# theori-io/nrsc5

Hardware: NVIDIA H100
Metric: cu8 I/Q Msamples/s (higher is better)
Workload: dtype u8/int16/f32

## Files before the change

### include/nrsc5_b200.h

```cpp
#ifndef NRSC5_B200_H
#define NRSC5_B200_H

#include <stddef.h>
#include <stdint.h>

#ifdef __cplusplus
extern "C" {
#endif

#define NRSC5B_MODE_FM 0
#define NRSC5B_MODE_AM 1

enum {
    NRSC5B_OK = 0,
    NRSC5B_ENODEV = -1,
    NRSC5B_EINVAL = -2,
    NRSC5B_ENOMEM = -3,
    NRSC5B_ECUDA = -4,
    NRSC5B_EFULL = -5,
    NRSC5B_EOVERFLOW = -6,
};

enum {
    NRSC5B_REC_FRAME = 1,
    NRSC5B_REC_PIDS = 2,
    NRSC5B_REC_SYNC = 3,
    NRSC5B_REC_LOST_SYNC = 4,
    NRSC5B_REC_MER = 5,
    NRSC5B_REC_BER = 6,
    NRSC5B_REC_SOFT_PM = 8,
    NRSC5B_REC_BLOCK = 9,
    NRSC5B_REC_PAD = 12,
    NRSC5B_REC_L2 = 20,
};

typedef struct nrsc5b_engine nrsc5b_engine_t;

typedef struct {
    int device;
    int nstreams;
    int mode;
    size_t input_capacity;
    size_t log_capacity;
    int emit_soft;
    int input_cs16;
} nrsc5b_config_t;

int nrsc5b_create(nrsc5b_engine_t **out, const nrsc5b_config_t *cfg);
void nrsc5b_destroy(nrsc5b_engine_t *e);
int nrsc5b_reset(nrsc5b_engine_t *e, int stream);
int nrsc5b_rewind(nrsc5b_engine_t *e);

int nrsc5b_set_cuda_stream(nrsc5b_engine_t *e, void *cuda_stream);

int nrsc5b_push_cu8(nrsc5b_engine_t *e, int stream, const uint8_t *buf, size_t nbytes);
int nrsc5b_push_cs16(nrsc5b_engine_t *e, int stream, const int16_t *buf, size_t nvalues);
int nrsc5b_push_cu8_all(nrsc5b_engine_t *e, const uint8_t *host, size_t host_stride, size_t nbytes);
int nrsc5b_push_cu8_device(nrsc5b_engine_t *e, int stream, const void *dev_buf, size_t nbytes);
int nrsc5b_attach_device_input(nrsc5b_engine_t *e, const void *dev_buf, size_t stride, size_t nbytes);

int nrsc5b_attach_device_log(nrsc5b_engine_t *e, void *dev_buf, size_t stride);

int nrsc5b_process(nrsc5b_engine_t *e);
int nrsc5b_process_available(nrsc5b_engine_t *e);
int nrsc5b_push_fence(nrsc5b_engine_t *e);
int nrsc5b_process_fence(nrsc5b_engine_t *e, int token);
int nrsc5b_prepare_async(nrsc5b_engine_t *e);
int nrsc5b_stage_cu8(nrsc5b_engine_t *e, int stream, const uint8_t *buf, size_t nbytes);
int nrsc5b_stage_cs16(nrsc5b_engine_t *e, int stream, const int16_t *buf, size_t nvalues);
int nrsc5b_submit(nrsc5b_engine_t *e, int flush);
int nrsc5b_poll(nrsc5b_engine_t *e, int wait);
const uint8_t *nrsc5b_batch_records(nrsc5b_engine_t *e, int stream, size_t *nbytes);

long nrsc5b_drain(nrsc5b_engine_t *e, int stream, uint8_t *out, size_t cap, size_t *needed);
int nrsc5b_drain_all(nrsc5b_engine_t *e, uint8_t *out, size_t out_stride, size_t *sizes);
int nrsc5b_take_overflow(nrsc5b_engine_t *e, int stream);
int nrsc5b_synchronize(nrsc5b_engine_t *e);

int nrsc5b_set_sync_state(nrsc5b_engine_t *e, int stream, int state);

typedef struct {
    uint64_t blocks;
    uint64_t samples;
    uint64_t p1_frames;
    uint64_t kernel_launches;
    uint64_t p1_fallbacks;
    uint64_t log_overflows;
} nrsc5b_stats_t;
int nrsc5b_get_stats(nrsc5b_engine_t *e, nrsc5b_stats_t *st);

int nrsc5b_set_profiling(nrsc5b_engine_t *e, int on);
int nrsc5b_get_kernel_times(nrsc5b_engine_t *e, double *ms4, unsigned long long *n4);

int nrsc5b_get_phase_cycles(nrsc5b_engine_t *e, unsigned long long *cyc12, unsigned long long *n12);

int nrsc5b_get_am_phase_cycles(nrsc5b_engine_t *e, unsigned long long *cyc12);

int nrsc5b_debug_set(int flags);

int nrsc5b_enable_l2(nrsc5b_engine_t *e, int on);

int nrsc5b_halfband_fm(int device, const uint8_t *cu8, size_t npairs, int16_t *out_ri);
int nrsc5b_viterbi_k7(int device, const int8_t *in, uint8_t *out, int len, int nframes);
int nrsc5b_viterbi_k7_ex(int device, const int8_t *in, uint8_t *out, int len, int nframes, int *fallbacks);
int nrsc5b_rs_decode(int device, uint8_t *blocks255, int *rc, int nblocks);
int nrsc5b_viterbi_k9(int device, const int8_t *in, uint8_t *out, int len, int njobs, unsigned g0, unsigned g1, unsigned g2,
                      int warmup, int chunk_warmup, int *rounds);
long nrsc5b_l2_frames(int device, const uint8_t *frames, size_t nbytes, uint8_t *out, size_t cap, size_t *needed);
int nrsc5b_fft2048(int device, const float *in, float *out, int nffts);

typedef struct nrsc5b_channelizer nrsc5b_channelizer_t;
int nrsc5b_chan_create(nrsc5b_channelizer_t **out, int device, const int *offsets_100khz, int nch);
void nrsc5b_chan_destroy(nrsc5b_channelizer_t *c);
int nrsc5b_chan_tables(nrsc5b_channelizer_t *c, int16_t *taps, int16_t *phasor);
int nrsc5b_chan_make_tables(const int *offsets_100khz, int nch, int16_t *taps, int16_t *phasor);
long long nrsc5b_chan_outputs(size_t nbytes);
int nrsc5b_chan_run_device(nrsc5b_channelizer_t *c, const void *d_cu8, size_t nbytes, void *d_out, size_t out_stride, void *cuda_stream);
int nrsc5b_chan_run(nrsc5b_channelizer_t *c, const uint8_t *cu8, size_t nbytes, int16_t *out);
int nrsc5b_chan_reset(nrsc5b_channelizer_t *c);
int nrsc5b_chan_push(nrsc5b_channelizer_t *c, const uint8_t *cu8, size_t nbytes, void *d_out, size_t out_stride, void *cuda_stream,
                     long long *nout);
int nrsc5b_chan_feed(nrsc5b_channelizer_t *c, nrsc5b_engine_t *e, const int *streams, const uint8_t *cu8, size_t nbytes);

int nrsc5b_chan_create_cs16(nrsc5b_channelizer_t **out, int device, const int *offsets_100khz, int nch);
int nrsc5b_chan_run_cs16(nrsc5b_channelizer_t *c, const int16_t *cs16, size_t nvalues, int16_t *out);
int nrsc5b_chan_run_device_cs16(nrsc5b_channelizer_t *c, const void *d_cs16, size_t nvalues, void *d_out, size_t out_stride,
                                void *cuda_stream);
int nrsc5b_chan_push_cs16(nrsc5b_channelizer_t *c, const int16_t *cs16, size_t nvalues, void *d_out, size_t out_stride,
                          void *cuda_stream, long long *nout);
int nrsc5b_chan_feed_cs16(nrsc5b_channelizer_t *c, nrsc5b_engine_t *e, const int *streams, const int16_t *cs16, size_t nvalues);

int nrsc5b_chan_create_am(nrsc5b_channelizer_t **out, int device, const int *offsets_10khz, int nch);
int nrsc5b_chan_create_am_cs16(nrsc5b_channelizer_t **out, int device, const int *offsets_10khz, int nch);
int nrsc5b_chan_make_tables_am(const int *offsets_10khz, int nch, int16_t *taps, int16_t *phasor);
long long nrsc5b_chan_outputs_am(size_t nbytes);

const char *nrsc5b_version(void);

#ifdef __cplusplus
}
#endif
#endif
```

### nrsc5_b200/csrc/engine.cu

```cuda
#include <cmath>
#include <cstdio>
#include <cstdlib>
#include <cstring>
#include <ctime>
#include <new>
#include <vector>

#include "../../include/nrsc5_b200.h"
#include "chan_feed.h"
#include "common.cuh"
#if defined(NB_EMU)
struct NvtxRange { explicit NvtxRange(const char *) {} };
#else
#include <nvtx3/nvToolsExt.h>
struct NvtxRange {
    explicit NvtxRange(const char *name) { nvtxRangePushA(name); }
    ~NvtxRange() { nvtxRangePop(); }
};
#endif
#include "rs.cuh"
#include "viterbi.cuh"
#include "viterbi_chunk.cuh"
#include "viterbi64.cuh"
#include "front.cuh"
// ... 1953 lines not shown
        }
    }
    CK(cudaStreamSynchronize(e->stream));
    return rc ? rc : (truncated ? NRSC5B_EOVERFLOW : NRSC5B_OK);
}

extern "C" int nrsc5b_take_overflow(nrsc5b_engine_t *e, int stream)
{
    if (!e || stream < 0 || stream >= e->dims.nstreams) return NRSC5B_EINVAL;
    const int v = e->overflowed[stream];
    e->overflowed[stream] = 0;
    return v;
}

extern "C" int nrsc5b_set_sync_state(nrsc5b_engine_t *e, int stream, int state)
{
    if (!e || stream < 0 || stream >= e->dims.nstreams || state < 0 || state > 2) return NRSC5B_EINVAL;
    CK(cudaMemcpyAsync(reinterpret_cast<uint8_t *>(e->dp.st + stream) + offsetof(StreamState, force_state), &state,
                       sizeof(int), cudaMemcpyHostToDevice, e->stream));
    CK(cudaStreamSynchronize(e->stream));
    return NRSC5B_OK;
}

extern "C" int nrsc5b_get_stats(nrsc5b_engine_t *e, nrsc5b_stats_t *out)
{
    if (!e || !out) return NRSC5B_EINVAL;
    CK(cudaStreamSynchronize(e->stream));
    const int S = e->dims.nstreams;
    CK(cudaMemcpy(e->h_state, e->dp.st, sizeof(StreamState) * S, cudaMemcpyDeviceToHost));
    unsigned long long frames = 0, samples = 0, blocks = 0, fb = 0;
    for (int s = 0; s < S; s++) {
        fb += e->h_state[s].p1_fallbacks;
        frames += e->h_state[s].frames_done;
        blocks += e->h_state[s].blocks_done;
        samples += (unsigned long long)(2 * e->h_state[s].start);
    }
    e->stats.p1_frames = frames;
    e->stats.p1_fallbacks = fb;
    e->stats.blocks = blocks;
    e->stats.samples = samples;
    *out = e->stats;
    return NRSC5B_OK;
}

static int use_device(int device)
{
    int ndev = 0;
    if (cudaGetDeviceCount(&ndev) != cudaSuccess || ndev <= 0 || device >= ndev) {
        fprintf(stderr, "nrsc5_b200: no usable CUDA device (the engine has no CPU path)\n");
        return NRSC5B_ENODEV;
    }
    if (cudaSetDevice(device) != cudaSuccess) return NRSC5B_ENODEV;
    return upload_tables(device);
}

extern "C" int nrsc5b_halfband_fm(int device, const uint8_t *cu8, size_t npairs, int16_t *out)
{
    int rc = use_device(device);
    if (rc) return rc;
    uint8_t *din = nullptr;
    short2 *dout = nullptr;
    CK(cudaMalloc(&din, 4 * npairs + 64));
    CK(cudaMalloc(&dout, npairs * sizeof(short2)));
    CK(cudaMemcpy(din, cu8, 4 * npairs, cudaMemcpyHostToDevice));
    launch_halfband_test(din, (long long)npairs, dout, 0);
    CK(cudaMemcpy(out, dout, npairs * sizeof(short2), cudaMemcpyDeviceToHost));
    cudaFree(din);
    cudaFree(dout);
    return NRSC5B_OK;
}

static int viterbi_k7_impl(int device, const int8_t *in, uint8_t *out, int len, int nframes, int *fallbacks);

extern "C" int nrsc5b_viterbi_k7(int device, const int8_t *in, uint8_t *out, int len, int nframes)
{
    return viterbi_k7_impl(device, in, out, len, nframes, nullptr);
}

extern "C" int nrsc5b_viterbi_k7_ex(int device, const int8_t *in, uint8_t *out, int len, int nframes, int *fallbacks)
{
    return viterbi_k7_impl(device, in, out, len, nframes, fallbacks);
}

static int viterbi_k7_impl(int device, const int8_t *in, uint8_t *out, int len, int nframes, int *fallbacks)
{
    int rc = use_device(device);
    if (rc) return rc;
    if (len < 32 || nframes <= 0) return NRSC5B_EINVAL;
    int8_t *din = nullptr;
    uint8_t *dout = nullptr;
    size_t nin = (size_t)nframes * 3 * len;
    CK(cudaMalloc(&din, nin));
    CK(cudaMalloc(&dout, (size_t)nframes * len));
    CK(cudaMemcpy(din, in, nin, cudaMemcpyHostToDevice));
    if (len >= 2048 && (len % 32) == 0) {
        const int total = len + 64;
        int *dflags = nullptr;
        CK(cudaMalloc(&dflags, (size_t)nframes * 3 * sizeof(int)));
        std::vector<int> fl(3 * (size_t)nframes, 0);
        for (int i = 0; i < nframes; i++) fl[i] = 1;
        CK(cudaMemcpy(dflags, fl.data(), fl.size() * sizeof(int), cudaMemcpyHostToDevice));
        uint32_t *dbw = nullptr;
        CK(cudaMalloc(&dbw, (size_t)nframes * (len / 32) * sizeof(uint32_t)));
        VitcArgs a;
        a.len = len;
        a.nch = (total + CH_LEN - 1) / CH_LEN;
        a.dec_stride = (size_t)a.nch * CH_LEN;
        a.ready_stride = 1;
        CK(cudaMalloc(&a.dec, (size_t)nframes * a.dec_stride * sizeof(uint2)));
        CK(cudaMalloc(&a.vspec, (size_t)nframes * a.nch * 16 * sizeof(uint2)));
        CK(cudaMalloc(&a.vend, (size_t)nframes * a.nch * 16 * sizeof(uint2)));
        CK(cudaMalloc(&a.tbend, (size_t)nframes * a.nch * sizeof(int)));
        CK(cudaMalloc(&a.hstate, (size_t)nframes * a.nch * sizeof(int)));
        a.vin = din;
        a.bitsw = dbw;
        a.ready = dflags + 2 * nframes;
        a.slow = dflags + nframes;
        V64Args b;
        b.vin = din;
        b.dec = a.dec;
        b.bitsw = dbw;
        b.ready = dflags;
        b.retry = dflags + 2 * nframes;
        b.stride = 1;
        b.len = len;
        b.ch = len >= 16384 ? 1024 : 256;
        b.nch = (total + b.ch - 1) / b.ch;
        b.dec_stride = a.dec_stride;
        CK(cudaMalloc(&b.vspec, (size_t)nframes * b.nch * 32 * sizeof(uint32_t)));
        CK(cudaMalloc(&b.vend, (size_t)nframes * b.nch * 32 * sizeof(uint32_t)));
        CK(cudaMalloc(&b.endstate, (size_t)nframes * sizeof(int)));
        CK(cudaFuncSetAttribute(k_vitc_emit, cudaFuncAttributeMaxDynamicSharedMemorySize, (int)vitc_emit_smem()));
        CK(cudaFuncSetAttribute(k_v64_emit, cudaFuncAttributeMaxDynamicSharedMemorySize, (int)V64_EMIT_SMEM));
        launch_v64(b, nframes, 0);
        launch_vitc(a, nframes, 0);
        {
            size_t nb = (size_t)nframes * len;
            k_vitc_unpack<<<(unsigned)((nb + 255) / 256), 256>>>(dbw, dout, nb);
        }
        CK(cudaDeviceSynchronize());
        CK(cudaMemcpy(fl.data(), dflags, fl.size() * sizeof(int), cudaMemcpyDeviceToHost));
        if (fallbacks) {
            *fallbacks = 0;
            for (int i = 0; i < nframes; i++) *fallbacks += fl[2 * (size_t)nframes + i] != 0;
        }
        cudaFree(a.dec); cudaFree(a.vspec); cudaFree(a.vend); cudaFree(a.tbend); cudaFree(a.hstate); cudaFree(dflags); cudaFree(dbw);
        cudaFree(b.vspec); cudaFree(b.vend); cudaFree(b.endstate);
    } else {
        uint2 *ddec = nullptr;
        CK(cudaMalloc(&ddec, (size_t)nframes * (len + 64) * sizeof(uint2)));
        k_viterbi_test<<<nframes, 32>>>(din, dout, ddec, len);
        CK(cudaDeviceSynchronize());
        cudaFree(ddec);
    }
    CK(cudaMemcpy(out, dout, (size_t)nframes * len, cudaMemcpyDeviceToHost));
    cudaFree(din);
    cudaFree(dout);
    return NRSC5B_OK;
}

extern "C" int nrsc5b_rs_decode(int device, uint8_t *blocks, int *rcs, int n)
{
    int rc = use_device(device);
    if (rc) return rc;
    uint8_t *db = nullptr;
    int *dr = nullptr;
// ... 127 lines not shown
```

### nrsc5_b200/csrc/viterbi64.cuh

```cuda
#pragma once
#include "common.cuh"
#include "viterbi_chunk.cuh"

namespace nb {

constexpr int V64_WARM = 256;
constexpr int V64_NORM = 32;
constexpr int V64_BIAS = 384;
constexpr int V64_WIN = 1024;
constexpr int V64_HEAD = 128;
constexpr int V64_GUESS = 64;

struct V64Args {
    const int8_t *vin;
    uint2 *dec;
    uint32_t *vspec;
    uint32_t *vend;
    int *endstate;
    uint32_t *bitsw;
    const int *ready;
    int *retry;
    int stride;
    int len;
    int ch;
    int nch;
    size_t dec_stride;
};

__device__ __forceinline__ unsigned v64_umax(unsigned a, unsigned b)
{
    unsigned r;
#if defined(NB_EMU)
    r = emu_max_u16x2(a, b);
#else
    asm("max.u16x2 %0, %1, %2;" : "=r"(r) : "r"(a), "r"(b));
#endif
    return r;
}
__device__ __forceinline__ unsigned v64_umin(unsigned a, unsigned b)
{
    unsigned r;
#if defined(NB_EMU)
    r = emu_min_u16x2(a, b);
#else
    asm("min.u16x2 %0, %1, %2;" : "=r"(r) : "r"(a), "r"(b));
#endif
    return r;
}
__device__ __forceinline__ unsigned v64_prmt(unsigned a, unsigned b, unsigned sel)
{
    unsigned r;
#if defined(NB_EMU)
    r = emu_prmt(a, b, sel);
#else
    asm("prmt.b32 %0, %1, %2, %3;" : "=r"(r) : "r"(a), "r"(b), "r"(sel));
#endif
    return r;
}

__host__ __device__ constexpr int v64_parity(unsigned v)
{
    return (int)((v ^ (v >> 1) ^ (v >> 2) ^ (v >> 3) ^ (v >> 4) ^ (v >> 5) ^ (v >> 6)) & 1u);
}
__host__ __device__ constexpr int v64_mp_index(int l)
{
    const unsigned reg = (unsigned)l << 1;
    const int k0 = v64_parity(reg & 0133u), k1 = v64_parity(reg & 0171u), k2 = v64_parity(reg & 0165u);
    const int u = (k1 && k2) ? 0 : (!k1 && !k2) ? 1 : (k1 && !k2) ? 2 : 3;
    return (k0 ? 0 : 4) | u;
}
__host__ __device__ constexpr int v64_mm_index(int l)
{
    const int i = v64_mp_index(l);
    return (i ^ 4) ^ 1;
}

struct V64State {
    unsigned P[32];

    __device__ __forceinline__ uint2 step(int s0, int s1, int s2)
    {
        const int c1 = V64_BIAS + s0, c2 = V64_BIAS - s0, b1 = s1 + s2, b2 = s1 - s2;
        unsigned M[8];
        M[0] = (unsigned)(c1 + b1) | ((unsigned)(c1 - b1) << 16);
        M[2] = (unsigned)(c1 + b2) | ((unsigned)(c1 - b2) << 16);
        M[4] = (unsigned)(c2 + b1) | ((unsigned)(c2 - b1) << 16);
        M[6] = (unsigned)(c2 + b2) | ((unsigned)(c2 - b2) << 16);
        M[1] = v64_prmt(M[0], 0, 0x1032);
        M[3] = v64_prmt(M[2], 0, 0x1032);
        M[5] = v64_prmt(M[4], 0, 0x1032);
        M[7] = v64_prmt(M[6], 0, 0x1032);
        unsigned N[32];
        unsigned w0 = 0, w1 = 0;
#pragma unroll
        for (int l = 0; l < 16; l++) {
            const unsigned E = P[2 * l], O = P[2 * l + 1];
            const unsigned Mp = M[v64_mp_index(l)], Mm = M[v64_mm_index(l)];
            const unsigned X1 = E + Mp, Y1 = O + Mm, X2 = E + Mm, Y2 = O + Mp;
            const unsigned N0 = v64_umax(X1, Y1), N1 = v64_umax(X2, Y2);
            const unsigned T1 = Y1 + 0x80008000u - X1, T2 = Y2 + 0x80008000u - X2;
            N[l] = v64_prmt(N0, N1, 0x5410);
            N[l + 16] = v64_prmt(N0, N1, 0x7632);
            const unsigned R = v64_prmt(T1, T2, 0xFDB9);
            if (l < 8) w0 |= R & (0x01010101u << (l & 7));
            else w1 |= R & (0x01010101u << (l & 7));
        }
#pragma unroll
        for (int i = 0; i < 32; i++) P[i] = N[i];
        return make_uint2(w0, w1);
    }

    __device__ __forceinline__ void normalise()
    {
        unsigned m = P[0];
#pragma unroll
        for (int i = 1; i < 32; i++) m = v64_umin(m, P[i]);
        m = v64_umin(m, v64_prmt(m, 0, 0x1032));
#pragma unroll
        for (int i = 0; i < 32; i++) P[i] -= m;
    }
};

__device__ __forceinline__ int v64_prev(int state, uint2 w)
{
    const unsigned word = (state & 8) ? w.y : w.x;
    return ((state << 1) & 62) | (int)((word >> (8 * (state >> 4) + (state & 7))) & 1u);
}

constexpr int V64_FWD_THREADS = 128;

__global__ void __launch_bounds__(V64_FWD_THREADS) k_v64_fwd(V64Args a)
{
    const int f = blockIdx.y;
    if (!a.ready[(size_t)f * a.stride]) return;
    const int c = blockIdx.x * V64_FWD_THREADS + threadIdx.x;
    if (c >= a.nch) return;
    const int total = a.len + 64;
    const int8_t *vin = a.vin + (size_t)f * 3 * a.len;
    uint2 *dec = a.dec + (size_t)f * a.dec_stride;
    const int s_begin = c * a.ch, s_end = min(total, s_begin + a.ch);
    const int sat_limit = 32767 - 12 * 381;
    int wsum = 0;
    bool bad = false;

    V64State vs;
#pragma unroll
    for (int i = 0; i < 32; i++) vs.P[i] = 0;

    auto fetch = [&](int g, uint32_t &x0, uint32_t &x1, uint32_t &x2) {
        if (g >= 0 && g < s_end) {
            int j = g + a.len - 32;
            if (j >= a.len) j -= a.len;
            if (j >= a.len) j -= a.len;
            const uint32_t *q = reinterpret_cast<const uint32_t *>(vin + 3 * (size_t)j);
            x0 = q[0]; x1 = q[1]; x2 = q[2];
        } else {
            x0 = x1 = x2 = 0;
        }
    };
    const int g_first = s_begin - V64_WARM;
    int wc = ((g_first % 79) + 79) % 79;
    uint32_t n0, n1, n2;
    fetch(g_first, n0, n1, n2);
#pragma unroll 1
    for (int g0 = g_first; g0 < s_end; g0 += 4) {
        const uint32_t sw[3] = { n0, n1, n2 };
        fetch(g0 + 4, n0, n1, n2);
        const bool store = g0 >= s_begin;
        uint2 held = make_uint2(0, 0);
#pragma unroll
        for (int k = 0; k < 4; k++) {
            auto sb = [&](int pos) -> int {
                const unsigned sel = (unsigned)(pos & 3) * 0x1111u | 0x8880u;
                return (int)v64_prmt(sw[pos >> 2], 0, sel);
            };
            const int s0 = sb(3 * k), s1 = sb(3 * k + 1), s2 = sb(3 * k + 2);
            wsum += abs(s0) + abs(s1) + abs(s2);
            if (wc == 0) {
                bad |= wsum > sat_limit;
                wsum = 0;
            }
            wc = wc == 78 ? 0 : wc + 1;
            const uint2 w = vs.step(s0, s1, s2);
            if (k & 1) {
                if (store) *reinterpret_cast<uint4 *>(dec + g0 + k - 1) = make_uint4(held.x, held.y, w.x, w.y);
            } else {
                held = w;
            }
        }
        if (((g0 + 4) & (V64_NORM - 1)) == 0) vs.normalise();
        if (g0 + 4 == s_begin) {
            uint32_t *o = a.vspec + ((size_t)f * a.nch + c) * 32;
#pragma unroll
            for (int i = 0; i < 32; i++) o[i] = vs.P[i];
        }
    }
    {
        uint32_t *o = a.vend + ((size_t)f * a.nch + c) * 32;
#pragma unroll
        for (int i = 0; i < 32; i++) o[i] = vs.P[i];
    }
    if (bad) atomicExch(&a.retry[(size_t)f * a.stride], 1);
}

constexpr int V64_CHECK_THREADS = 256;

__global__ void __launch_bounds__(V64_CHECK_THREADS) k_v64_check(V64Args a)
{
    const int f = blockIdx.x;
    if (!a.ready[(size_t)f * a.stride]) return;
    const int lane = threadIdx.x & 31, warp = threadIdx.x >> 5, nwarps = V64_CHECK_THREADS / 32;
    const uint32_t *vspec = a.vspec + (size_t)f * a.nch * 32, *vend = a.vend + (size_t)f * a.nch * 32;
    bool ok = true;
    for (int c = 1 + warp; c < a.nch; c += nwarps) {
        const unsigned x = vend[(size_t)(c - 1) * 32 + lane], y = vspec[(size_t)c * 32 + lane];
        const int xr = (int)(__shfl_sync(0xffffffffu, x, 0) & 0xffff), yr = (int)(__shfl_sync(0xffffffffu, y, 0) & 0xffff);
        ok &= ((int)(x & 0xffff) - xr == (int)(y & 0xffff) - yr) && ((int)(x >> 16) - xr == (int)(y >> 16) - yr);
    }
    if (!__all_sync(0xffffffffu, ok) && lane == 0) atomicExch(&a.retry[(size_t)f * a.stride], 1);
    if (warp == 0) {
        const unsigned x = vend[(size_t)(a.nch - 1) * 32 + lane];
        int v = (int)(x & 0xffff), idx = lane;
        const int v2 = (int)(x >> 16);
        if (v2 > v) { v = v2; idx = lane + 32; }
#pragma unroll
        for (int o = 16; o; o >>= 1) {
            const int ov = __shfl_xor_sync(0xffffffffu, v, o), oi = __shfl_xor_sync(0xffffffffu, idx, o);
            if (ov > v || (ov == v && oi < idx)) { v = ov; idx = oi; }
        }
        if (lane == 0) a.endstate[f] = idx;
    }
}

constexpr int V64_EMIT_WARPS = 4;
constexpr int V64_EMIT_STEPS = V64_WIN + V64_HEAD;
constexpr int V64_EMIT_LD = V64_EMIT_STEPS + V64_EMIT_STEPS / 32 + 1;
constexpr size_t V64_EMIT_SMEM = (size_t)V64_EMIT_WARPS * V64_EMIT_LD * sizeof(uint2);
__device__ __forceinline__ int v64_pad(int q) { return q + (q >> 5); }

__global__ void __launch_bounds__(V64_EMIT_WARPS * 32) k_v64_emit(V64Args a)
{
#if defined(NB_EMU)
    unsigned char *v64_smem = emu::dyn_smem();
#else
    extern __shared__ __align__(16) unsigned char v64_smem[];
#endif
    const int f = blockIdx.y;
    if (!a.ready[(size_t)f * a.stride]) return;
    const int lane = threadIdx.x & 31, warp = threadIdx.x >> 5;
    const int total = a.len + 64;
    const int w = blockIdx.x * V64_EMIT_WARPS + warp;
    const int lo = w * V64_WIN;
    if (lo >= total) return;
    uint2 *sd = reinterpret_cast<uint2 *>(v64_smem) + (size_t)warp * V64_EMIT_LD;
    const uint2 *dec = a.dec + (size_t)f * a.dec_stride + lo;
    const int n = min(total - lo, V64_WIN);
    const int nst = min(total - lo, V64_EMIT_STEPS);
    for (int i = lane; i < nst; i += 32) sd[v64_pad(i)] = dec[i];
    __syncwarp();
    auto walk = [&](int state, int from, int to) {
        for (int q = from; q > to; q--) state = v64_prev(state, sd[v64_pad(q)]);
        return state;
    };
    int true_end;
    if (nst == n) {
        true_end = a.endstate[f];
    } else {
        bool merged = false;
        int ref = 0;
        for (int look = min(V64_HEAD / 2, nst - n); ; look = nst - n) {
            int e0 = lane, e1 = lane + 32;
            for (int q = n + look - 1; q > n - 1; q--) {
                const uint2 w = sd[v64_pad(q)];
                e0 = v64_prev(e0, w);
// ... 47 lines not shown
```

### nrsc5_b200/engine.py

```python
from __future__ import annotations

import ctypes
import os
import struct

import numpy as np

_HERE = os.path.dirname(os.path.abspath(__file__))

REC_FRAME, REC_PIDS, REC_SYNC, REC_LOST_SYNC, REC_MER, REC_BER = 1, 2, 3, 4, 5, 6
REC_SOFT_PM, REC_BLOCK = 8, 9
REC_PAD = 12
REC_L2 = 20
EV_SERVICE, EV_ALIGN, EV_AAS, EV_PACKET = 16, 17, 18, 19
L2F_LOST, L2F_EV_OVERFLOW = 1, 2


class EngineError(RuntimeError):
    pass


class _Config(ctypes.Structure):
    _fields_ = [("device", ctypes.c_int), ("nstreams", ctypes.c_int), ("mode", ctypes.c_int),
                ("input_capacity", ctypes.c_size_t), ("log_capacity", ctypes.c_size_t),
                ("emit_soft", ctypes.c_int), ("input_cs16", ctypes.c_int)]


class Stats(ctypes.Structure):
    _fields_ = [("blocks", ctypes.c_uint64), ("samples", ctypes.c_uint64),
                ("p1_frames", ctypes.c_uint64), ("kernel_launches", ctypes.c_uint64),
                ("p1_fallbacks", ctypes.c_uint64), ("log_overflows", ctypes.c_uint64)]


def lib_path() -> str:
    return os.path.join(_HERE, "libnrsc5_b200.so")


_lib = None


def load_library():
    global _lib
    if _lib is not None:
        return _lib
    p = lib_path()
    if not os.path.exists(p):
        raise EngineError(f"{p} is missing: build it with `python -c 'import __graft_entry__ as g; g.build()'` "
                          "(there is no CPU fallback)")
    L = ctypes.CDLL(p)
    vp, sz, ci = ctypes.c_void_p, ctypes.c_size_t, ctypes.c_int
    L.nrsc5b_version.restype = ctypes.c_char_p
    L.nrsc5b_create.argtypes = [ctypes.POINTER(vp), ctypes.POINTER(_Config)]
    L.nrsc5b_destroy.argtypes = [vp]
    L.nrsc5b_destroy.restype = None
    L.nrsc5b_reset.argtypes = [vp, ci]
    L.nrsc5b_rewind.argtypes = [vp]
    L.nrsc5b_set_profiling.argtypes = [vp, ci]
    L.nrsc5b_get_kernel_times.argtypes = [vp, vp, vp]
    L.nrsc5b_get_phase_cycles.argtypes = [vp, vp, vp]
    L.nrsc5b_get_am_phase_cycles.argtypes = [vp, vp]
    L.nrsc5b_set_cuda_stream.argtypes = [vp, vp]
    L.nrsc5b_push_cu8.argtypes = [vp, ci, vp, sz]
    L.nrsc5b_push_cs16.argtypes = [vp, ci, vp, sz]
    L.nrsc5b_push_cu8_device.argtypes = [vp, ci, vp, sz]
    L.nrsc5b_push_cu8_all.argtypes = [vp, vp, sz, sz]
    L.nrsc5b_attach_device_input.argtypes = [vp, vp, sz, sz]
    L.nrsc5b_attach_device_log.argtypes = [vp, vp, sz]
    L.nrsc5b_process.argtypes = [vp]
    L.nrsc5b_process_available.argtypes = [vp]
    L.nrsc5b_push_fence.argtypes = [vp]
    L.nrsc5b_process_fence.argtypes = [vp, ci]
    L.nrsc5b_synchronize.argtypes = [vp]
    L.nrsc5b_prepare_async.argtypes = [vp]
    L.nrsc5b_stage_cu8.argtypes = [vp, ci, vp, sz]
    L.nrsc5b_stage_cs16.argtypes = [vp, ci, vp, sz]
    L.nrsc5b_submit.argtypes = [vp, ci]
    L.nrsc5b_poll.argtypes = [vp, ci]
    L.nrsc5b_batch_records.argtypes = [vp, ci, ctypes.POINTER(sz)]
    L.nrsc5b_batch_records.restype = vp
    L.nrsc5b_drain.argtypes = [vp, ci, vp, sz, ctypes.POINTER(sz)]
    L.nrsc5b_drain.restype = ctypes.c_long
    L.nrsc5b_drain_all.argtypes = [vp, vp, sz, vp]
    L.nrsc5b_set_sync_state.argtypes = [vp, ci, ci]
    L.nrsc5b_take_overflow.argtypes = [vp, ci]
    L.nrsc5b_get_stats.argtypes = [vp, ctypes.POINTER(Stats)]
    L.nrsc5b_enable_l2.argtypes = [vp, ci]
    L.nrsc5b_l2_frames.argtypes = [ci, ctypes.c_char_p, sz, vp, sz, ctypes.POINTER(sz)]
    L.nrsc5b_l2_frames.restype = ctypes.c_long
    L.nrsc5b_halfband_fm.argtypes = [ci, vp, sz, vp]
    L.nrsc5b_viterbi_k7.argtypes = [ci, vp, vp, ci, ci]
    L.nrsc5b_viterbi_k7_ex.argtypes = [ci, vp, vp, ci, ci, ctypes.POINTER(ci)]
    L.nrsc5b_rs_decode.argtypes = [ci, vp, vp, ci]
    L.nrsc5b_fft2048.argtypes = [ci, vp, vp, ci]
    _lib = L
    return L


def _check(rc, what):
    if rc < 0:
        names = {-1: "ENODEV (no CUDA device; no CPU path exists)", -2: "EINVAL", -3: "ENOMEM", -4: "ECUDA", -5: "EFULL",
                 -6: "EOVERFLOW (a stream's record log overflowed: raise log_capacity)"}
        raise EngineError(f"{what} failed: {names.get(rc, rc)}")
    return rc


def parse_l2(pay: bytes) -> dict:
    frame_off, lc, nbits, pci, flags, pdu_len, ev_len, ordinal = struct.unpack_from("<8I", pay, 0)
    ev = pay[32:32 + ev_len]
    pdu = bytes(pay[32 + ev_len:32 + ev_len + pdu_len])
    events, off = [], 0
    while off < len(ev):
        ty, plen = struct.unpack_from("<II", ev, off)
        p = ev[off + 8: off + 8 + plen]
        off += 8 + ((plen + 3) & ~3)
        if ty == EV_SERVICE:
            k = ("program", "access", "type", "codec_mode", "blend_control", "gain", "common_delay", "latency")
            r = dict(zip(k, struct.unpack("<8i", p[:32])))
        elif ty == EV_ALIGN:
            r = dict(zip(("program", "stream_id", "offset"), struct.unpack("<3I", p[:12])))
        elif ty == EV_AAS:
            r = {"data": bytes(p)}
        elif ty == EV_PACKET:
            prog, sid, seq, shape, fl, size, at = struct.unpack("<7I", p[:28])
            r = {"program": prog, "stream_id": sid, "seq": seq, "shape": shape, "flags": fl, "size": size,
                 "data": pdu[at:at + size]}
        else:
            raise EngineError(f"corrupt L2 event stream (type {ty})")
        events.append((ty, r))
    return {"frame_off": frame_off, "lc": lc, "nbits": nbits, "pci": pci, "flags": flags, "ordinal": ordinal,
            "pdu": pdu, "events": events}


def with_l2_in_call_order(raw: bytes):
    offs = []
    records = parse_records(raw, offs)
    l2_of = {r["frame_rec_off"]: r for ty, r in records if ty == REC_L2}
    out = []
    for (ty, r), at in zip(records, offs):
        if ty == REC_L2:
            continue
        out.append((ty, r))
        if ty == REC_FRAME and at in l2_of:
            out.extend(l2_of[at]["events"])
    return out


def parse_records(raw: bytes, offsets: list = None):
    out = []
    off, n = 0, len(raw)
    while off < n:
        ty, plen = struct.unpack_from("<II", raw, off)
        if ty == REC_PAD:
            off += 8 + ((plen + 3) & ~3)
            continue
        if offsets is not None:
            offsets.append(off)
        pay = raw[off + 8: off + 8 + plen]
        off += 8 + ((plen + 3) & ~3)
        if ty == REC_FRAME:
            lc, nbits = struct.unpack_from("<II", pay, 0)
            rec = {"lc": lc, "nbits": nbits, "bits": bytes(pay[8:])}
        elif ty == REC_PIDS:
            rec = {"bits": bytes(pay[:10]), "crc_ok": (pay[10] if len(pay) > 10 else None)}
        elif ty == REC_SYNC:
            f, psmi = struct.unpack_from("<fi", pay)
            flags = struct.unpack_from("<4i", pay, 8) if len(pay) >= 24 else (-1, -1, -1, -1)
            rec = {"freq_offset": f, "psmi": psmi, "flags": list(flags)}
        elif ty == REC_LOST_SYNC:
            rec = {}
        elif ty == REC_MER:
            lo, up = struct.unpack("<ff", pay)
            rec = {"lower": lo, "upper": up}
        elif ty == REC_BER:
            rec = {"cber": struct.unpack("<f", pay)[0]}
# ... 118 lines not shown

    def process_fence(self, token: int):
        _check(self._L.nrsc5b_process_fence(self._h, token), "nrsc5b_process_fence")

    def stage_cu8(self, stream: int, samples) -> int:
        a = np.ascontiguousarray(np.frombuffer(samples, dtype=np.uint8) if isinstance(samples, (bytes, bytearray)) else samples,
                                 dtype=np.uint8)
        rc = self._L.nrsc5b_stage_cu8(self._h, stream, a.ctypes.data if a.size else None, a.size)
        if rc != -5:
            _check(rc, "nrsc5b_stage_cu8")
        return rc

    def submit(self, flush: bool = False) -> int:
        return _check(self._L.nrsc5b_submit(self._h, int(flush)), "nrsc5b_submit")

    def poll(self, wait: bool = False) -> int:
        return _check(self._L.nrsc5b_poll(self._h, int(wait)), "nrsc5b_poll")

    def batch_records(self, stream: int):
        n = ctypes.c_size_t(0)
        ptr = self._L.nrsc5b_batch_records(self._h, stream, ctypes.byref(n))
        if self._L.nrsc5b_take_overflow(self._h, stream) and not self.allow_overflow:
            raise EngineError(f"stream {stream}: record log overflowed (log_capacity too small)")
        return parse_records(ctypes.string_at(ptr, n.value)) if ptr and n.value else []

    def synchronize(self):
        _check(self._L.nrsc5b_synchronize(self._h), "nrsc5b_synchronize")

    def drain_raw(self, stream: int) -> bytes:
        need = ctypes.c_size_t(0)
        buf = ctypes.create_string_buffer(self._log_cap)
        n = self._L.nrsc5b_drain(self._h, stream, buf, self._log_cap, ctypes.byref(need))
        _check(n, "nrsc5b_drain")
        if self._L.nrsc5b_take_overflow(self._h, stream) and not self.allow_overflow:
            raise EngineError(f"stream {stream}: record log overflowed (log_capacity too small); the drained records are a prefix")
        return buf.raw[:n]

    def drain(self, stream: int):
        return parse_records(self.drain_raw(stream))

    def drain_all_raw(self, out: np.ndarray = None):
        if out is None:
            out = np.empty((self.nstreams, self._log_cap), dtype=np.uint8)
        sizes = (ctypes.c_size_t * self.nstreams)()
        rc = self._L.nrsc5b_drain_all(self._h, out.ctypes.data, out.strides[0], sizes)
        if not (rc == -6 and self.allow_overflow):
            _check(rc, "nrsc5b_drain_all")
        return [out[s, :sizes[s]] for s in range(self.nstreams)]

    def drain_all(self):
        return [parse_records(r.tobytes()) for r in self.drain_all_raw()]

    def enable_l2(self, on: bool = True):
        _check(self._L.nrsc5b_enable_l2(self._h, int(on)), "nrsc5b_enable_l2")

    def set_sync_state(self, stream: int, state: int):
        _check(self._L.nrsc5b_set_sync_state(self._h, stream, state), "nrsc5b_set_sync_state")

    def stats(self) -> Stats:
        st = Stats()
        _check(self._L.nrsc5b_get_stats(self._h, ctypes.byref(st)), "nrsc5b_get_stats")
        return st


def halfband_fm(cu8: np.ndarray, device: int = 0) -> np.ndarray:
    a = np.ascontiguousarray(cu8, dtype=np.uint8)
    n = a.size // 4
    out = np.empty(2 * n, dtype=np.int16)
    _check(load_library().nrsc5b_halfband_fm(device, a.ctypes.data, n, out.ctypes.data), "nrsc5b_halfband_fm")
    return out


def viterbi_k7(soft: np.ndarray, length: int, device: int = 0, want_fallbacks: bool = False):
    s = np.ascontiguousarray(soft, dtype=np.int8)
    nframes = s.size // (3 * length)
    out = np.empty(nframes * length, dtype=np.uint8)
    fb = ctypes.c_int(0)
    _check(load_library().nrsc5b_viterbi_k7_ex(device, s.ctypes.data, out.ctypes.data, length, nframes, ctypes.byref(fb)),
           "nrsc5b_viterbi_k7_ex")
    out = out.reshape(nframes, length)
    return (out, fb.value) if want_fallbacks else out


def l2_frames(frames, device: int = 0, cap: int = 64 << 20):
    blob = bytearray()
    for f in frames:
        if f is None:
            blob += struct.pack("<II", 0, 0)
        else:
            lc, nbits, bits = f
            nb = (nbits + 7) // 8
            blob += struct.pack("<II", lc, nbits) + bytes(bits[:nb]) + bytes((-nb) % 4)
    out = ctypes.create_string_buffer(cap)
    need = ctypes.c_size_t(0)
    n = load_library().nrsc5b_l2_frames(device, bytes(blob), len(blob), out, cap, ctypes.byref(need))
    _check(n, "nrsc5b_l2_frames")
    return [r for t, r in parse_records(out.raw[:n]) if t == REC_L2]


def rs_decode(blocks: np.ndarray, device: int = 0):
    b = np.ascontiguousarray(blocks, dtype=np.uint8).reshape(-1, 255).copy()
    rc = np.empty(b.shape[0], dtype=np.int32)
    _check(load_library().nrsc5b_rs_decode(device, b.ctypes.data, rc.ctypes.data, b.shape[0]), "nrsc5b_rs_decode")
    return rc, b


def viterbi_k9(sym: np.ndarray, gens=(0o561, 0o657, 0o711), warmup: int = 0, chunk_warmup: int = 0, device: int = 0):
    a = np.ascontiguousarray(sym, dtype=np.int8)
    a = a.reshape(1, -1) if a.ndim == 1 else a
    njobs, n = a.shape[0], a.shape[1] // 3
    out = np.empty((njobs, n), dtype=np.uint8)
    rounds = np.empty(njobs, dtype=np.int32)
    L = load_library()
    L.nrsc5b_viterbi_k9.argtypes = [ctypes.c_int, ctypes.c_void_p, ctypes.c_void_p, ctypes.c_int, ctypes.c_int, ctypes.c_uint,
                                    ctypes.c_uint, ctypes.c_uint, ctypes.c_int, ctypes.c_int, ctypes.c_void_p]
    _check(L.nrsc5b_viterbi_k9(device, a.ctypes.data, out.ctypes.data, n, njobs, *gens, warmup, chunk_warmup, rounds.ctypes.data),
           "nrsc5b_viterbi_k9")
    return out, rounds & 0xffff, rounds >> 16


def fft2048(x: np.ndarray, device: int = 0) -> np.ndarray:
    a = np.ascontiguousarray(x, dtype=np.complex64).reshape(-1, 2048)
    out = np.empty_like(a)
    _check(load_library().nrsc5b_fft2048(device, a.ctypes.data, out.ctypes.data, a.shape[0]), "nrsc5b_fft2048")
    return out
```

Measured before the change: 161,800.

## Restructure K7 Viterbi ACS with in-place state layout, fused add-max, and grouped fetch

Rewrites the 64-state Viterbi butterfly step so it is templated on a rotating state-layout phase J. This avoids per-step permutes of path metrics and uses the fused __viaddmax_u16x2 instruction for add-compare-select. Branch metrics are built with sign flips chosen at compile time. The input fetch is widened to groups of 8 steps, and the saturation window sum is computed per group with byte abs and dp4a instead of per step. It also adds a standalone viterbi_k7_fast test entry point, at the cost of more complex decision-bit packing and larger unrolled code that raises register pressure.

Measured after the change: 169,600 (median of 6 runs). +4.8%, better.

```diff
diff --git a/include/nrsc5_b200.h b/include/nrsc5_b200.h
--- a/include/nrsc5_b200.h
+++ b/include/nrsc5_b200.h
@@ -103,6 +103,7 @@
 int nrsc5b_halfband_fm(int device, const uint8_t *cu8, size_t npairs, int16_t *out_ri);
 int nrsc5b_viterbi_k7(int device, const int8_t *in, uint8_t *out, int len, int nframes);
 int nrsc5b_viterbi_k7_ex(int device, const int8_t *in, uint8_t *out, int len, int nframes, int *fallbacks);
+int nrsc5b_viterbi_k7_fast(int device, const int8_t *in, int len, int nframes, int ch, uint32_t *dec, int *retry);
 int nrsc5b_rs_decode(int device, uint8_t *blocks255, int *rc, int nblocks);
 int nrsc5b_viterbi_k9(int device, const int8_t *in, uint8_t *out, int len, int njobs, unsigned g0, unsigned g1, unsigned g2,
                       int warmup, int chunk_warmup, int *rounds);
diff --git a/nrsc5_b200/csrc/engine.cu b/nrsc5_b200/csrc/engine.cu
--- a/nrsc5_b200/csrc/engine.cu
+++ b/nrsc5_b200/csrc/engine.cu
@@ -2059,6 +2059,44 @@
     return viterbi_k7_impl(device, in, out, len, nframes, fallbacks);
 }
 
+extern "C" int nrsc5b_viterbi_k7_fast(int device, const int8_t *in, int len, int nframes, int ch, uint32_t *dec, int *retry)
+{
+    int rc = use_device(device);
+    if (rc) return rc;
+    if (len < 32 || (len % 32) || nframes <= 0 || ch < 32 || (ch % 32)) return NRSC5B_EINVAL;
+    const int total = len + 64;
+    V64Args b;
+    b.stride = 1;
+    b.len = len;
+    b.ch = ch;
+    b.nch = (total + ch - 1) / ch;
+    b.dec_stride = (size_t)total;
+    int8_t *din = nullptr;
+    int *dflags = nullptr;
+    CK(cudaMalloc(&din, (size_t)nframes * 3 * len));
+    CK(cudaMemcpy(din, in, (size_t)nframes * 3 * len, cudaMemcpyHostToDevice));
+    std::vector<int> fl(2 * (size_t)nframes, 0);
+    for (int i = 0; i < nframes; i++) fl[i] = 1;
+    CK(cudaMalloc(&dflags, fl.size() * sizeof(int)));
+    CK(cudaMemcpy(dflags, fl.data(), fl.size() * sizeof(int), cudaMemcpyHostToDevice));
+    b.vin = din;
+    b.ready = dflags;
+    b.retry = dflags + nframes;
+    CK(cudaMalloc(&b.dec, (size_t)nframes * total * sizeof(uint2)));
+    CK(cudaMalloc(&b.bitsw, (size_t)nframes * (len / 32) * sizeof(uint32_t)));
+    CK(cudaMalloc(&b.vspec, (size_t)nframes * b.nch * 32 * sizeof(uint32_t)));
+    CK(cudaMalloc(&b.vend, (size_t)nframes * b.nch * 32 * sizeof(uint32_t)));
+    CK(cudaMalloc(&b.endstate, (size_t)nframes * sizeof(int)));
+    CK(cudaFuncSetAttribute(k_v64_emit, cudaFuncAttributeMaxDynamicSharedMemorySize, (int)V64_EMIT_SMEM));
+    launch_v64(b, nframes, 0);
+    CK(cudaDeviceSynchronize());
+    CK(cudaMemcpy(dec, b.dec, (size_t)nframes * total * sizeof(uint2), cudaMemcpyDeviceToHost));
+    CK(cudaMemcpy(retry, b.retry, (size_t)nframes * sizeof(int), cudaMemcpyDeviceToHost));
+    cudaFree(din); cudaFree(dflags); cudaFree(b.dec); cudaFree(b.bitsw);
+    cudaFree(b.vspec); cudaFree(b.vend); cudaFree(b.endstate);
+    return NRSC5B_OK;
+}
+
 static int viterbi_k7_impl(int device, const int8_t *in, uint8_t *out, int len, int nframes, int *fallbacks)
 {
     int rc = use_device(device);
diff --git a/nrsc5_b200/csrc/viterbi64.cuh b/nrsc5_b200/csrc/viterbi64.cuh
--- a/nrsc5_b200/csrc/viterbi64.cuh
+++ b/nrsc5_b200/csrc/viterbi64.cuh
@@ -1,4 +1,6 @@
 #pragma once
+#include <type_traits>
+#include <utility>
 #include "common.cuh"
 #include "viterbi_chunk.cuh"
 
@@ -6,6 +8,7 @@
 
 constexpr int V64_WARM = 256;
 constexpr int V64_NORM = 32;
+constexpr int V64_GROUP = 8;
 constexpr int V64_BIAS = 384;
 constexpr int V64_WIN = 1024;
 constexpr int V64_HEAD = 128;
@@ -27,87 +30,127 @@
     size_t dec_stride;
 };
 
-__device__ __forceinline__ unsigned v64_umax(unsigned a, unsigned b)
+__device__ __forceinline__ unsigned v64_umin(unsigned a, unsigned b)
 {
     unsigned r;
 #if defined(NB_EMU)
-    r = emu_max_u16x2(a, b);
-#else
-    asm("max.u16x2 %0, %1, %2;" : "=r"(r) : "r"(a), "r"(b));
+    r = emu_min_u16x2(a, b);
+#else
+    asm("min.u16x2 %0, %1, %2;" : "=r"(r) : "r"(a), "r"(b));
 #endif
     return r;
 }
-__device__ __forceinline__ unsigned v64_umin(unsigned a, unsigned b)
+__device__ __forceinline__ unsigned v64_prmt(unsigned a, unsigned b, unsigned sel)
 {
     unsigned r;
 #if defined(NB_EMU)
-    r = emu_min_u16x2(a, b);
-#else
-    asm("min.u16x2 %0, %1, %2;" : "=r"(r) : "r"(a), "r"(b));
+    r = emu_prmt(a, b, sel);
+#else
+    asm("prmt.b32 %0, %1, %2, %3;" : "=r"(r) : "r"(a), "r"(b), "r"(sel));
 #endif
     return r;
 }
-__device__ __forceinline__ unsigned v64_prmt(unsigned a, unsigned b, unsigned sel)
-{
-    unsigned r;
-#if defined(NB_EMU)
-    r = emu_prmt(a, b, sel);
-#else
-    asm("prmt.b32 %0, %1, %2, %3;" : "=r"(r) : "r"(a), "r"(b), "r"(sel));
-#endif
+__device__ __forceinline__ unsigned v64_addmax(unsigned a, unsigned b, unsigned c)
+{
+#if defined(NB_EMU)
+    return emu_max_u16x2(emu_add_s16x2(a, b), c);
+#else
+    return __viaddmax_u16x2(a, b, c);
+#endif
+}
+__device__ __forceinline__ unsigned v64_absb4(unsigned x)
+{
+#if defined(NB_EMU)
+    unsigned r = 0;
+    for (int i = 0; i < 4; i++) {
+        const int v = (int8_t)(x >> (8 * i));
+        r |= (unsigned)(v < 0 ? -v : v) << (8 * i);
+    }
     return r;
+#else
+    return __vabsdiffs4(x, 0u);
+#endif
 }
 
 __host__ __device__ constexpr int v64_parity(unsigned v)
 {
     return (int)((v ^ (v >> 1) ^ (v >> 2) ^ (v >> 3) ^ (v >> 4) ^ (v >> 5) ^ (v >> 6)) & 1u);
 }
-__host__ __device__ constexpr int v64_mp_index(int l)
-{
-    const unsigned reg = (unsigned)l << 1;
-    const int k0 = v64_parity(reg & 0133u), k1 = v64_parity(reg & 0171u), k2 = v64_parity(reg & 0165u);
-    const int u = (k1 && k2) ? 0 : (!k1 && !k2) ? 1 : (k1 && !k2) ? 2 : 3;
-    return (k0 ? 0 : 4) | u;
-}
-__host__ __device__ constexpr int v64_mm_index(int l)
-{
-    const int i = v64_mp_index(l);
-    return (i ^ 4) ^ 1;
+__host__ __device__ constexpr int v64_neg(int b)
+{
+    const unsigned reg = (unsigned)b << 1;
+    return (v64_parity(reg & 0133u) ? 0 : 4) | (v64_parity(reg & 0171u) ? 0 : 2) | (v64_parity(reg & 0165u) ? 0 : 1);
+}
+
+__host__ __device__ constexpr int v64_state(int J, int reg, int half)
+{
+    const int x = reg | (half << 5);
+    int n = 0;
+    for (int k = 0; k < 6; k++) n |= ((x >> ((k + J) % 6)) & 1) << k;
+    return n;
 }
 
 struct V64State {
     unsigned P[32];
 
+    template <int J>
     __device__ __forceinline__ uint2 step(int s0, int s1, int s2)
     {
-        const int c1 = V64_BIAS + s0, c2 = V64_BIAS - s0, b1 = s1 + s2, b2 = s1 - s2;
+        constexpr int H = 5 - J;
+        constexpr int flip = (((0133 >> H) & 1) << 2) | (((0171 >> H) & 1) << 1) | ((0165 >> H) & 1);
         unsigned M[8];
-        M[0] = (unsigned)(c1 + b1) | ((unsigned)(c1 - b1) << 16);
-        M[2] = (unsigned)(c1 + b2) | ((unsigned)(c1 - b2) << 16);
-        M[4] = (unsigned)(c2 + b1) | ((unsigned)(c2 - b1) << 16);
-        M[6] = (unsigned)(c2 + b2) | ((unsigned)(c2 - b2) << 16);
-        M[1] = v64_prmt(M[0], 0, 0x1032);
-        M[3] = v64_prmt(M[2], 0, 0x1032);
-        M[5] = v64_prmt(M[4], 0, 0x1032);
-        M[7] = v64_prmt(M[6], 0, 0x1032);
+#pragma unroll
+        for (int m = 0; m < 8; m++) {
+            const int v0 = (m & 4) ? -s0 : s0, v1 = (m & 2) ? -s1 : s1, v2 = (m & 1) ? -s2 : s2;
+            const int com = V64_BIAS + ((flip & 4) ? 0 : v0) + ((flip & 2) ? 0 : v1) + ((flip & 1) ? 0 : v2);
+            const int dif = ((flip & 4) ? v0 : 0) + ((flip & 2) ? v1 : 0) + ((flip & 1) ? v2 : 0);
+            M[m] = (unsigned)com * 0x10001u + (unsigned)dif * 0xFFFF0001u;
+        }
+        auto acc_of = [](int n) -> int {
+            return J == 0 ? (n >> 3) & 1 : J == 1 ? (n >> 4) & 1 : ((n >> 3) & 1) | (((n >> 4) & 1) << 1);
+        };
+        auto byte_of = [](int n) -> int {
+            return J == 0 ? n >> 4 : J == 1 ? ((n >> 5) & 1) | (((n >> 3) & 1) << 1)
+                                            : (((n >> 5) & 1) << 1) | ((n >> (4 - J)) & 1);
+        };
+        unsigned A[4] = { 0, 0, 0, 0 };
         unsigned N[32];
-        unsigned w0 = 0, w1 = 0;
 #pragma unroll
         for (int l = 0; l < 16; l++) {
-            const unsigned E = P[2 * l], O = P[2 * l + 1];
-            const unsigned Mp = M[v64_mp_index(l)], Mm = M[v64_mm_index(l)];
-            const unsigned X1 = E + Mp, Y1 = O + Mm, X2 = E + Mm, Y2 = O + Mp;
-            const unsigned N0 = v64_umax(X1, Y1), N1 = v64_umax(X2, Y2);
-            const unsigned T1 = Y1 + 0x80008000u - X1, T2 = Y2 + 0x80008000u - X2;
-            N[l] = v64_prmt(N0, N1, 0x5410);
-            N[l + 16] = v64_prmt(N0, N1, 0x7632);
-            const unsigned R = v64_prmt(T1, T2, 0xFDB9);
-            if (l < 8) w0 |= R & (0x01010101u << (l & 7));
-            else w1 |= R & (0x01010101u << (l & 7));
+            const int rE = ((l >> J) << (J + 1)) | (l & ((1 << J) - 1)), rO = rE | (1 << J);
+            const unsigned E = P[rE], O = P[rO];
+            const int b = v64_state(J, rE, 0) >> 1, bh = v64_state(J, rE, 1) >> 1;
+            const unsigned Mp = M[v64_neg(b)], Mm = M[v64_neg(b) ^ 7];
+            const unsigned Y1 = O + Mm, Y2 = O + Mp;
+            const unsigned N0 = v64_addmax(E, Mp, Y1), N1 = v64_addmax(E, Mm, Y2);
+            const unsigned T1 = Y1 + 0x80008000u - N0, T2 = Y2 + 0x80008000u - N1;
+            const int st[4] = { b, bh, b | 32, bh | 32 };
+            unsigned sel = 0, mask = 0;
+#pragma unroll
+            for (int i = 0; i < 4; i++) {
+                sel |= (unsigned)(9 + 2 * i) << (4 * byte_of(st[i]));
+                mask |= 1u << (8 * byte_of(st[i]) + (st[i] & 7));
+            }
+            A[acc_of(b)] |= v64_prmt(T1, T2, sel) & mask;
+            if constexpr (J < 3) {
+                N[rE] = N0;
+                N[rO] = N1;
+            } else {
+                N[b] = v64_prmt(N0, N1, 0x5410);
+                N[bh] = v64_prmt(N0, N1, 0x7632);
+            }
         }
 #pragma unroll
         for (int i = 0; i < 32; i++) P[i] = N[i];
-        return make_uint2(w0, w1);
+        if constexpr (J == 0) {
+            return make_uint2(A[0], A[1]);
+        } else if constexpr (J == 1) {
+            return make_uint2(v64_prmt(A[0], A[1], 0x5140), v64_prmt(A[0], A[1], 0x7362));
+        } else {
+#pragma unroll
+            for (int i = 0; i < 4; i++) A[i] *= 0x101u;
+            return make_uint2(v64_prmt(A[0], A[2], 0x7351), v64_prmt(A[1], A[3], 0x7351));
+        }
     }
 
     __device__ __forceinline__ void normalise()
@@ -125,6 +168,12 @@
 {
     const unsigned word = (state & 8) ? w.y : w.x;
     return ((state << 1) & 62) | (int)((word >> (8 * (state >> 4) + (state & 7))) & 1u);
+}
+
+template <class F, int... K>
+__device__ __forceinline__ void v64_unroll(F &f, std::integer_sequence<int, K...>)
+{
+    (f(std::integral_constant<int, K>{}), ...);
 }
 
 constexpr int V64_FWD_THREADS = 128;
@@ -147,49 +196,72 @@
 #pragma unroll
     for (int i = 0; i < 32; i++) vs.P[i] = 0;
 
-    auto fetch = [&](int g, uint32_t &x0, uint32_t &x1, uint32_t &x2) {
+    static_assert(V64_GROUP % 4 == 0 && 32 % V64_GROUP == 0 && V64_WARM % V64_GROUP == 0 && V64_NORM % V64_GROUP == 0,
+                  "groups are whole layout cycles and tile chunks (multiples of 32 steps), the warm-up and V64_NORM");
+    constexpr int GW = 3 * V64_GROUP / 4;
+    const uint32_t *vw = reinterpret_cast<const uint32_t *>(vin);
+    const int fw = 3 * a.len / 4;
+    auto fetch = [&](int g, int &jw, uint32_t (&x)[GW]) {
         if (g >= 0 && g < s_end) {
-            int j = g + a.len - 32;
-            if (j >= a.len) j -= a.len;
-            if (j >= a.len) j -= a.len;
-            const uint32_t *q = reinterpret_cast<const uint32_t *>(vin + 3 * (size_t)j);
-            x0 = q[0]; x1 = q[1]; x2 = q[2];
+#pragma unroll
+            for (int i = 0; i < GW; i++) x[i] = vw[jw + i];
         } else {
-            x0 = x1 = x2 = 0;
-        }
+#pragma unroll
+            for (int i = 0; i < GW; i++) x[i] = 0;
+        }
+        jw = jw + GW >= fw ? jw + GW - fw : jw + GW;
     };
     const int g_first = s_begin - V64_WARM;
     int wc = ((g_first % 79) + 79) % 79;
-    uint32_t n0, n1, n2;
-    fetch(g_first, n0, n1, n2);
+    int jw = 3 * (((g_first - 32) % a.len + a.len) % a.len) / 4;
+    uint32_t nw[GW];
+    fetch(g_first, jw, nw);
 #pragma unroll 1
-    for (int g0 = g_first; g0 < s_end; g0 += 4) {
-        const uint32_t sw[3] = { n0, n1, n2 };
-        fetch(g0 + 4, n0, n1, n2);
+    for (int g0 = g_first; g0 < s_end; g0 += V64_GROUP) {
+        uint32_t sw[GW];
+#pragma unroll
+        for (int i = 0; i < GW; i++) sw[i] = nw[i];
+        fetch(g0 + V64_GROUP, jw, nw);
         const bool store = g0 >= s_begin;
+        uint32_t u[GW];
+        int gsum = 0;
+#pragma unroll
+        for (int i = 0; i < GW; i++) {
+            u[i] = v64_absb4(sw[i]);
+            gsum = (int)__dp4a(u[i], 0x01010101u, (unsigned)gsum);
+        }
+        if (wc == 0 || wc > 79 - V64_GROUP) {
+            const int nb = 3 * (wc == 0 ? 1 : 80 - wc);
+            int head = 0;
+#pragma unroll
+            for (int i = 0; i < GW; i++) {
+                const int k = min(max(nb - 4 * i, 0), 4);
+                head = (int)__dp4a(u[i], k ? 0x01010101u >> (8 * (4 - k)) : 0u, (unsigned)head);
+            }
+            bad |= wsum + head > sat_limit;
+            wsum = gsum - head;
+        } else {
+            wsum += gsum;
+        }
+        wc = wc + V64_GROUP >= 79 ? wc + V64_GROUP - 79 : wc + V64_GROUP;
         uint2 held = make_uint2(0, 0);
-#pragma unroll
-        for (int k = 0; k < 4; k++) {
+        auto one = [&](auto kc) {
+            constexpr int k = decltype(kc)::value;
             auto sb = [&](int pos) -> int {
                 const unsigned sel = (unsigned)(pos & 3) * 0x1111u | 0x8880u;
                 return (int)v64_prmt(sw[pos >> 2], 0, sel);
             };
             const int s0 = sb(3 * k), s1 = sb(3 * k + 1), s2 = sb(3 * k + 2);
-            wsum += abs(s0) + abs(s1) + abs(s2);
-            if (wc == 0) {
-                bad |= wsum > sat_limit;
-                wsum = 0;
-            }
-            wc = wc == 78 ? 0 : wc + 1;
-            const uint2 w = vs.step(s0, s1, s2);
+            const uint2 w = vs.template step<k % 4>(s0, s1, s2);
             if (k & 1) {
                 if (store) *reinterpret_cast<uint4 *>(dec + g0 + k - 1) = make_uint4(held.x, held.y, w.x, w.y);
             } else {
                 held = w;
             }
-        }
-        if (((g0 + 4) & (V64_NORM - 1)) == 0) vs.normalise();
-        if (g0 + 4 == s_begin) {
+        };
+        v64_unroll(one, std::make_integer_sequence<int, V64_GROUP>{});
+        if (((g0 + V64_GROUP) & (V64_NORM - 1)) == 0) vs.normalise();
+        if (g0 + V64_GROUP == s_begin) {
             uint32_t *o = a.vspec + ((size_t)f * a.nch + c) * 32;
 #pragma unroll
             for (int i = 0; i < 32; i++) o[i] = vs.P[i];
diff --git a/nrsc5_b200/engine.py b/nrsc5_b200/engine.py
--- a/nrsc5_b200/engine.py
+++ b/nrsc5_b200/engine.py
@@ -90,6 +90,7 @@
     L.nrsc5b_halfband_fm.argtypes = [ci, vp, sz, vp]
     L.nrsc5b_viterbi_k7.argtypes = [ci, vp, vp, ci, ci]
     L.nrsc5b_viterbi_k7_ex.argtypes = [ci, vp, vp, ci, ci, ctypes.POINTER(ci)]
+    L.nrsc5b_viterbi_k7_fast.argtypes = [ci, vp, ci, ci, ci, vp, vp]
     L.nrsc5b_rs_decode.argtypes = [ci, vp, vp, ci]
     L.nrsc5b_fft2048.argtypes = [ci, vp, vp, ci]
     _lib = L
@@ -374,6 +375,16 @@
     return (out, fb.value) if want_fallbacks else out
 
 
+def viterbi_k7_fast(soft: np.ndarray, length: int, chunk: int, device: int = 0):
+    s = np.ascontiguousarray(soft, dtype=np.int8)
+    nframes = s.size // (3 * length)
+    dec = np.empty((nframes, length + 64, 2), dtype=np.uint32)
+    retry = np.empty(nframes, dtype=np.int32)
+    _check(load_library().nrsc5b_viterbi_k7_fast(device, s.ctypes.data, length, nframes, chunk, dec.ctypes.data,
+                                                 retry.ctypes.data), "nrsc5b_viterbi_k7_fast")
+    return dec, retry != 0
+
+
 def l2_frames(frames, device: int = 0, cap: int = 64 << 20):
     blob = bytearray()
     for f in frames:
```
